# JuliaSmoothOptimizers/Krylov.jl

Measured on AMD Instinct MI355X. Metric: cg_iters_per_sec_poisson3d_csr_512cubed, higher is better.
Workload: dtype f64

## Files before the change

krylov.jl_amd/csrc/api.cpp:

```cpp
#include <cmath>
#include <cstdlib>

#include "khip_internal.hpp"

using namespace khip;

extern "C" int khip_comm_destroy_internal(khip_ctx *ctx);

namespace khip {
enum MapOpHost { H_COPY = 0, H_FILL, H_SCAL, H_SCALCOPY, H_DIVCOPY, H_AXPY, H_AXPBY, H_REF, H_WAXPY, H_VMUL, H_VDIV };
constexpr int kPadHost = 8;
}

namespace khip {
static int g_optional_build_failures = 0;
void optional_build(int rc) {
  if (rc == KHIP_OK) return;
  const hipError_t e = (hipError_t)take_hip_error();
  (void)hipGetLastError();
  if (e == hipErrorOutOfMemory || e == hipErrorMemoryAllocation) return;
  ++g_optional_build_failures;
  fprintf(stderr, "libkrylov_hip: an optional accelerator build failed (%d: %s; HIP: %s) -- falling back to the plain kernels\n", rc,
          khip_last_error(), hipGetErrorString(e));
}
// ... 100 lines not shown
  KHIP_CHECK_HIP(hipGetDeviceProperties(&prop, device));
  ctx->num_cu = prop.multiProcessorCount > 0 ? prop.multiProcessorCount : 256;
  KHIP_TRY(ensure_reduction_scratch(ctx, 1 << 18, 1));
  KHIP_CHECK_HIP(hipMalloc(&ctx->results, sizeof(double) * kResultSlots));
  KHIP_CHECK_HIP(hipMalloc(&ctx->results_dd, sizeof(dd) * kResultSlots));
  KHIP_CHECK_HIP(hipMemset(ctx->results, 0, sizeof(double) * kResultSlots));
  KHIP_CHECK_HIP(hipMemset(ctx->results_dd, 0, sizeof(dd) * kResultSlots));
  KHIP_CHECK_HIP(hipHostMalloc(reinterpret_cast<void **>(&ctx->results_pinned), sizeof(double) * kResultSlots * 2,
                               hipHostMallocDefault));
  *out = ctx;
  return KHIP_OK;
}

int khip_ctx_destroy(khip_ctx *ctx) {
  if (!ctx) return KHIP_OK;
  (void)hipSetDevice(ctx->device);
  (void)hipStreamSynchronize(ctx->stream);
  khip_comm_destroy_internal(ctx);
  panel_scratch_destroy(ctx);
  for (hipEvent_t e : ctx->prof_events) (void)hipEventDestroy(e);
  (void)hipFree(ctx->partials);
  (void)hipFree(ctx->partials2);
  (void)hipFree(ctx->tickets);
  (void)hipFree(ctx->results);
  (void)hipFree(ctx->results_dd);
  (void)hipHostFree(ctx->results_pinned);
  if (ctx->ev_fetch) (void)hipEventDestroy(ctx->ev_fetch);
  if (ctx->ev_red) (void)hipEventDestroy(ctx->ev_red);
  for (int i = 0; i < khip_ctx::kEvRing; ++i) {
    if (ctx->ev_a[i]) (void)hipEventDestroy(ctx->ev_a[i]);
    if (ctx->ev_b[i]) (void)hipEventDestroy(ctx->ev_b[i]);
  }
  if (ctx->comm_stream_hi && ctx->comm_stream_hi != ctx->comm_stream_lo) (void)hipStreamDestroy(ctx->comm_stream_hi);
  if (ctx->comm_stream_lo) (void)hipStreamDestroy(ctx->comm_stream_lo);
  if (ctx->own_stream) (void)hipStreamDestroy(ctx->stream);
  delete ctx;
  return KHIP_OK;
}

int khip_ctx_sync(khip_ctx *ctx) {
  KHIP_REQUIRE(ctx, "ctx_sync: null context");
  KHIP_CHECK_HIP(hipStreamSynchronize(ctx->stream));
  return KHIP_OK;
}

void *khip_ctx_stream(khip_ctx *ctx) { return ctx ? ctx->stream : nullptr; }

static int *tuning_field(khip_ctx *ctx, const char *key) {
  Tuning &t = ctx->tune;
  struct { const char *k; int *p; } tab[] = {
      {"spmv_kernel", &t.spmv_kernel}, {"spmv_rows", &t.spmv_rows}, {"spmv_vec", &t.spmv_vec},
      {"spmv_nt", &t.spmv_nt},         {"spmv_xcd", &t.spmv_xcd},   {"spmv_lanes", &t.spmv_lanes},
      {"compensated", &t.compensated}, {"nt_min_elems", &t.nt_min_elems}, {"overlap_halo", &t.overlap_halo},
      {"profile_spmv", &t.profile_spmv}, {"comm_priority", &t.comm_priority}, {"spmv_persist", &t.spmv_persist}, {"spmv_nty", &t.spmv_nty}, {"spmv_dot_early", &t.spmv_dot_early}, {"spmv_codes", &t.spmv_codes}, {"spmv_delta", &t.spmv_delta}, {"spmv_blk_pub", &t.spmv_blk_pub}, {"spmv_sell", &t.spmv_sell}, {"spmv_sell_narrow", &t.spmv_sell_narrow}, {"spmv_sell_entries", &t.spmv_sell_entries}, {"spmv_sell_pair", &t.spmv_sell_pair}, {"cg_setup_fused", &t.cg_setup_fused}, {"cg_defer_x", &t.cg_defer_x}, {"spmv_wide", &t.spmv_wide}, {"spmv_tiles", &t.spmv_tiles}, {"spmv_cap", &t.spmv_cap}, {"spmv_template", &t.spmv_template}, {"spmv_tmpl_rows", &t.spmv_tmpl_rows}, {"mgs_keep", &t.mgs_keep}, {"spmm_sweep", &t.spmm_sweep}, {"spmm_win_sweep", &t.spmm_win_sweep}, {"spmm_wide", &t.spmm_wide}, {"panel_fuse", &t.panel_fuse}, {"panel_signs", &t.panel_signs}, {"panel_qr_tsqr", &t.panel_qr_tsqr}, {"panel_a_lds", &t.panel_a_lds}, {"panel_nt", &t.panel_nt}, {"gmres_sstep", &t.gmres_sstep}, {"panel_multi_tiles", &t.panel_multi_tiles}, {"ilu_blocks", &t.ilu_blocks}, {"ilu_grid", &t.ilu_grid}, {"halo_mode", &t.halo_mode}, {"halo_gather_pct", &t.halo_gather_pct}, {"spmm_window", &t.spmm_window}, {"spmm_tile", &t.spmm_tile}, {"spmm_tile_exp", &t.spmm_tile_exp}, {"spmm_tile_nt", &t.spmm_tile_nt}, {"spmm_tile_slices", &t.spmm_tile_slices}, {"spmm_tile_pencil", &t.spmm_tile_pencil}, {"spmm_tile_slide", &t.spmm_tile_slide}, {"spmm_tile_ahead", &t.spmm_tile_ahead}, {"spmm_tile_xcd", &t.spmm_tile_xcd}, {"spmm_tile_dbuf", &t.spmm_tile_dbuf}, {"spmm_tile_pair", &t.spmm_tile_pair}, {"spmm_tile_waves", &t.spmm_tile_waves}, {"spmm_tile_grid", &t.spmm_tile_grid}, {"spmm_tile_shape", &t.spmm_tile_shape}, {"spmm_window_grid", &t.spmm_window_grid}, {"spmm_sweep_s", &t.spmm_sweep_s}, {"spmm_sweep_w", &t.spmm_sweep_w}, {"red_u", &t.red_u}, {"hist_window", &t.hist_window}};
  for (auto &e : tab)
    if (strcmp(e.k, key) == 0) return e.p;
  return nullptr;
}

int khip_ctx_set_option(khip_ctx *ctx, const char *key, int value) {
  KHIP_REQUIRE(ctx && key, "set_option: null argument");
  int *p = tuning_field(ctx, key);
  KHIP_REQUIRE(p, "set_option: unknown key '%s'", key);
  *p = value;
  if (p == &ctx->tune.comm_priority) {
    KHIP_CHECK_HIP(hipStreamSynchronize(ctx->stream));
    KHIP_CHECK_HIP(hipStreamSynchronize(ctx->comm_stream_hi));
    KHIP_CHECK_HIP(hipStreamSynchronize(ctx->comm_stream_lo));
    ctx->comm_stream = value ? ctx->comm_stream_hi : ctx->comm_stream_lo;
  }
  return KHIP_OK;
}

int khip_ctx_get_option(khip_ctx *ctx, const char *key, int *value) {
  KHIP_REQUIRE(ctx && key && value, "get_option: null argument");
  int *p = tuning_field(ctx, key);
  KHIP_REQUIRE(p, "get_option: unknown key '%s'", key);
  *value = *p;
  return KHIP_OK;
}

int khip_malloc(khip_ctx *ctx, size_t bytes, void **dptr) {
  KHIP_REQUIRE(ctx && dptr, "malloc: null argument");
  KHIP_CHECK_HIP(hipSetDevice(ctx->device));
  *dptr = nullptr;
  if (bytes == 0) return KHIP_OK;
  KHIP_CHECK_HIP(hipMalloc(dptr, bytes));
  return KHIP_OK;
}

int khip_free(khip_ctx *ctx, void *dptr) {
  KHIP_REQUIRE(ctx, "free: null context");
  if (!dptr) return KHIP_OK;
  KHIP_CHECK_HIP(hipStreamSynchronize(ctx->stream));
  KHIP_CHECK_HIP(hipFree(dptr));
  return KHIP_OK;
}

int khip_memcpy_h2d(khip_ctx *ctx, void *dst, const void *src_host, size_t bytes) {
  KHIP_REQUIRE(ctx && (bytes == 0 || (dst && src_host)), "memcpy_h2d: null argument");
  if (!bytes) return KHIP_OK;
  KHIP_CHECK_HIP(hipMemcpyAsync(dst, src_host, bytes, hipMemcpyHostToDevice, ctx->stream));
  KHIP_CHECK_HIP(hipStreamSynchronize(ctx->stream));
  return KHIP_OK;
}

int khip_memcpy_d2h(khip_ctx *ctx, void *dst_host, const void *src, size_t bytes) {
// ... 563 lines not shown
```

krylov.jl_amd/csrc/device_reduce.hpp:

```cpp
#pragma once

#include <hip/hip_runtime.h>

#include "khip_internal.hpp"
#include "solver_device.hpp"

namespace khip {

typedef double dbl2 __attribute__((ext_vector_type(2)));
template <int VEC> struct VecT;
template <> struct VecT<1> { using type = double; };
template <> struct VecT<2> { using type = dbl2; };

__device__ __forceinline__ double vget(const double &v, int) { return v; }
__device__ __forceinline__ double vget(const dbl2 &v, int i) { return i == 0 ? v.x : v.y; }
__device__ __forceinline__ void vset(double &v, int, double s) { v = s; }
__device__ __forceinline__ void vset(dbl2 &v, int i, double s) { if (i == 0) v.x = s; else v.y = s; }

template <bool NT, typename T> __device__ __forceinline__ T ldg(const T *p) {
  if (NT) return __builtin_nontemporal_load(p);
  return *p;
}
template <bool NT, typename T> __device__ __forceinline__ void stg(T v, T *p) {
  if (NT) __builtin_nontemporal_store(v, p);
// ... 40 lines not shown
__device__ __forceinline__ double dpp_f64(double v) {
  int lo = __double2loint(v), hi = __double2hiint(v);
  lo = __builtin_amdgcn_update_dpp(0, lo, CTRL, ROW_MASK, 0xf, false);
  hi = __builtin_amdgcn_update_dpp(0, hi, CTRL, ROW_MASK, 0xf, false);
  return __hiloint2double(hi, lo);
}
template <int CTRL, int ROW_MASK>
__device__ __forceinline__ dd dpp_step(dd v) {
  dd o;
  o.hi = dpp_f64<CTRL, ROW_MASK>(v.hi);
  o.lo = dpp_f64<CTRL, ROW_MASK>(v.lo);
  return dd_merge(v, o);
}

constexpr int kResultLane = 63;

__device__ __forceinline__ dd wave_reduce(dd v) {
#ifdef KHIP_REDUCE_SHFL
#pragma unroll
  for (int off = 1; off < 64; off <<= 1) {
    dd o;
    o.hi = __shfl_up(v.hi, off, 64);
    o.lo = __shfl_up(v.lo, off, 64);
    if ((int)(threadIdx.x & 63) < off) o = dd{0.0, 0.0};
    v = dd_merge(v, o);
  }
  return v;
#endif
  v = dpp_step<0x111, 0xf>(v);
  v = dpp_step<0x112, 0xf>(v);
  v = dpp_step<0x114, 0xf>(v);
  v = dpp_step<0x118, 0xf>(v);
  v = dpp_step<0x142, 0xa>(v);
  v = dpp_step<0x143, 0xc>(v);
  return v;
}

struct RedArgs {
  dd *wave_partials;
  dd *blk_partials;
  unsigned *ticket;
  double *results;
  dd *results_dd;
  int64_t cap;
  int64_t wave_offset;
  int slot;
  const long long *stop_seq;
  long long seq;
  int epi;
  void *epi_state;
};

template <int NOUT>
__device__ __forceinline__ void wave_publish(dd (&acc)[NOUT], const RedArgs &ra) {
  const int64_t wid = ra.wave_offset + (int64_t)blockIdx.x * (blockDim.x >> 6) + (threadIdx.x >> 6);
#pragma unroll
  for (int o = 0; o < NOUT; ++o) {
    dd r = wave_reduce(acc[o]);
    if ((threadIdx.x & 63) == kResultLane) ra.wave_partials[(size_t)o * ra.cap + wid] = r;
  }
}

template <int NOUT>
__device__ __forceinline__ void block_publish(dd (&acc)[NOUT], const RedArgs &ra, dd *s_red) {
  const int tid = threadIdx.x, lane = tid & 63, wave = tid >> 6;
  const int64_t wid = ra.wave_offset + (int64_t)blockIdx.x * (blockDim.x >> 6) + wave;
#pragma unroll
  for (int o = 0; o < NOUT; ++o) s_red[o * kBlock + tid] = acc[o];
  __syncthreads();
  if (wave == 0) {
#pragma unroll
    for (int o = 0; o < NOUT; ++o) {
      dd v = s_red[o * kBlock + lane];
      v = dd_merge(v, s_red[o * kBlock + 64 + lane]);
      v = dd_merge(v, s_red[o * kBlock + 128 + lane]);
      v = dd_merge(v, s_red[o * kBlock + 192 + lane]);
      v = wave_reduce(v);
      if (lane == kResultLane) ra.wave_partials[(size_t)o * ra.cap + wid] = v;
    }
  } else if (lane == kResultLane) {
#pragma unroll
    for (int o = 0; o < NOUT; ++o) ra.wave_partials[(size_t)o * ra.cap + wid] = dd{0.0, 0.0};
  }
}

template <int NOUT>
__device__ __forceinline__ void block_reduce(dd (&acc)[NOUT], dd (*s_w)[kWavesPerBlock]) {
  const int lane = threadIdx.x & 63, wave = threadIdx.x >> 6;
#pragma unroll
  for (int o = 0; o < NOUT; ++o) {
    dd r = wave_reduce(acc[o]);
    if (lane == kResultLane) s_w[o][wave] = r;
  }
  __syncthreads();
  if (threadIdx.x == 0) {
#pragma unroll
    for (int o = 0; o < NOUT; ++o) {
      dd t = s_w[o][0];
#pragma unroll
      for (int w = 1; w < kWavesPerBlock; ++w) t = dd_merge(t, s_w[o][w]);
      acc[o] = t;
    }
  }
}

template <int NOUT>
__global__ __launch_bounds__(kBlock) void reduce_finish_kernel(RedArgs ra, int64_t P) {
  __shared__ dd s_w[NOUT][kWavesPerBlock];
  __shared__ int s_last;
  if (seq_skip(ra.stop_seq, ra.seq)) return;
  const int G = gridDim.x;
  const int64_t chunk = (P + G - 1) / G;
  const int64_t lo = chunk * blockIdx.x;
  const int64_t hi = (lo + chunk < P) ? lo + chunk : P;
  dd acc[NOUT];
#pragma unroll
  for (int o = 0; o < NOUT; ++o) {
    dd a = {0.0, 0.0};
    const dd *src = ra.wave_partials + (size_t)o * ra.cap;
    for (int64_t base = lo + threadIdx.x; base < hi; base += (int64_t)kBlock * 8) {
      dd v[8];
#pragma unroll
      for (int j = 0; j < 8; ++j) {
        const int64_t i = base + (int64_t)j * kBlock;
        v[j] = src[i < hi ? i : base];
      }
#pragma unroll
      for (int j = 0; j < 8; ++j)
        if (base + (int64_t)j * kBlock < hi) a = dd_merge(a, v[j]);
    }
    acc[o] = a;
  }
  block_reduce<NOUT>(acc, s_w);
  if (G == 1) {
    if (threadIdx.x == 0) {
#pragma unroll
      for (int o = 0; o < NOUT; ++o) {
// ... 65 lines not shown
```

krylov.jl_amd/csrc/khip_internal.hpp:

```cpp
#pragma once

#include <hip/hip_runtime.h>

#include <unistd.h>

#include <chrono>
#include <cstdarg>
#include <cstdint>
#include <cstdio>
#include <cstring>
#include <string>
#include <vector>

#include "../../include/krylov_hip.h"

namespace khip {

void set_error(const char *fmt, ...);
void note_hip_error(int e);
int take_hip_error();

inline void klogf(int fd, const char *fmt, ...) {
  va_list ap;
  va_start(ap, fmt);
// ... 8 lines not shown
    hipError_t e__ = (expr);                                                              \
    if (e__ != hipSuccess) {                                                              \
      ::khip::note_hip_error((int)e__);                                                   \
      ::khip::set_error("%s failed: %s (%s:%d)", #expr, hipGetErrorString(e__), __FILE__, \
                        __LINE__);                                                        \
      return KHIP_ERR_HIP;                                                                \
    }                                                                                     \
  } while (0)

#define KHIP_REQUIRE(cond, ...)          \
  do {                                   \
    if (!(cond)) {                       \
      ::khip::set_error(__VA_ARGS__);    \
      return KHIP_ERR_INVALID;           \
    }                                    \
  } while (0)

#define KHIP_TRY(expr)                 \
  do {                                 \
    int rc__ = (expr);                 \
    if (rc__ != KHIP_OK) return rc__;  \
  } while (0)

struct dd {
  double hi, lo;
};

__host__ __device__ inline double dd_value(double hi, double lo) { return __builtin_isfinite(hi) ? hi + lo : hi; }

constexpr int kMaxNout = 4;
constexpr int kMaxRedOut = 64;
constexpr int kResultSlots = 256;

struct Comm;

struct Tuning {
  int spmv_kernel = 0;
  int spmv_rows = 256;
  int spmv_vec = 1;
  int spmv_nt = 0;
  int spmv_xcd = 0;
  int spmv_nty = -1;
  int spmv_dot_early = 0;
  int spmv_tiles = 1;
  int spmv_template = 1;
  int spmv_tmpl_rows = 8;
  int spmv_cap = 0;
  int cg_defer_x = 1;
  int cg_setup_fused = 1;
  int spmv_sell = 2;
  int spmv_sell_pair = 1;
  int spmv_sell_entries = 1;
  int spmv_sell_narrow = 0;
  int spmv_blk_pub = 0;
  int spmv_delta = 0;
  int spmv_wide = 0;
  int spmv_codes = 1;
  int spmv_lanes = 0;
  int spmv_persist = 0;
  int compensated = 1;
  int nt_min_elems = 1 << 22;
  int mgs_keep = -1;
  int hist_window = 1 << 14;
  int red_u = 0;
  int ilu_blocks = 1;
  int ilu_grid = 0;
  int panel_multi_tiles = 2;
  int gmres_sstep = 4;
  int panel_nt = 0;
  int panel_a_lds = 1;
  int panel_qr_tsqr = 0;
  int panel_signs = 1;
  int panel_fuse = 1;
  int spmm_wide = 1;
  int spmm_window_grid = 0;
  int spmm_tile = 1;
  int spmm_tile_exp = 0;
  int spmm_tile_waves = 0;
  int spmm_tile_grid = 0;
  int spmm_tile_pair = 1;
  int spmm_tile_dbuf = -1;
  int spmm_tile_xcd = -1;
  int spmm_tile_ahead = 0;
  int spmm_tile_slide = -1;
  int spmm_tile_pencil = 0;
  int spmm_tile_slices = 0;
  int spmm_tile_nt = 0;
  int spmm_tile_shape = 0;
  int spmm_window = 1;
  int spmm_sweep = 0;
  int spmm_win_sweep = 0;
  int spmm_sweep_s = 0;
  int spmm_sweep_w = 64;
  int overlap_halo = 1;
  int halo_mode = 0;
  int halo_gather_pct = 50;
  int halo_self = 0;
  int comm_priority = 1;
  int profile_spmv = 0;
};

struct SeqCtl {
  const long long *stop_seq = nullptr;
  long long seq = 0;
  int epi = 0;
  void *epi_state = nullptr;
};

struct LanczosEpi {
  const double *coef = nullptr;
  const double *r1 = nullptr;
  int sub_r1 = 0;
};

}

namespace khip {
enum SpmmLast {
  kSlFamily = 0,
  kSlL, kSlNL, kSlDbuf, kSlAhead, kSlRunLen, kSlGrid, kSlXcd, kSlLaunches, kSlDirect,
  kSlSweepS, kSlSweepW, kSlSweepK, kSlSweepCols, kSlNt, kSlDist, kSlP, kSlPow2, kSlBlock, kSlLds, kSlNumCu,
  kSpmmLastWords = 24
};
}

struct khip_ctx {
  int device = 0;
  hipStream_t stream = nullptr;
  bool own_stream = false;
  hipStream_t comm_stream = nullptr;
  hipStream_t comm_stream_hi = nullptr, comm_stream_lo = nullptr;
  static constexpr int kEvRing = 16;
  hipEvent_t ev_a[kEvRing] = {}, ev_b[kEvRing] = {};
  unsigned ev_cur = 0;
  hipEvent_t ev_fetch = nullptr;
  hipEvent_t ev_red = nullptr;
  bool allreduce_pending = false;
  int num_cu = 256;
  int64_t spmm_last[khip::kSpmmLastWords] = {};
  khip::dd *partials = nullptr;
  khip::dd *partials2 = nullptr;
  unsigned *tickets = nullptr;
  int64_t red_cap1 = 0;
  int *scratch_word = nullptr;
  double *results = nullptr;
  khip::dd *results_dd = nullptr;
  double *results_pinned = nullptr;
  int next_slot = 0;
  khip::Tuning tune;
  khip::SeqCtl ctl;
  khip::LanczosEpi lz;
  khip::Comm *comm = nullptr;
  void *panel_scratch = nullptr;
  std::vector<hipEvent_t> prof_events;
  std::vector<int> prof_tags;
  int prof_spmv_tag = 0;
  size_t prof_used = 0;
};

struct khip_csr {
  khip_ctx *ctx = nullptr;
  int64_t m = 0, n = 0, nnz = 0;
  int32_t *rowptr = nullptr;
  int32_t *blockptr = nullptr;
  int32_t *col = nullptr;
  double *val = nullptr;
  int64_t max_row_nnz = 0;
  int64_t band = 0;
  int64_t plane_rows = 0;
  int64_t line_rows = 0;
  double mean_row_nnz = 0;
  bool dist = false;
  int64_t n_global = 0, row0 = 0;
  int64_t n_ghost = 0;
  double *ghost = nullptr;
  double *sendbuf = nullptr;
  int32_t *send_idx = nullptr;
  double *ghost_w = nullptr, *sendbuf_w = nullptr;
  int halo_w_cap = 0;
  int64_t n_send = 0;
  std::vector<int64_t> send_off, recv_off;
  std::vector<int64_t> part_starts;
  std::vector<int32_t> ghost_gid;
  bool self_halo = false;
  bool gather = false;
  int64_t gather_maxm = 0;
  std::vector<int64_t> gather_rows;
  int64_t interior_lo = 0, interior_hi = 0;
  uint16_t *tmpl_id = nullptr;
  int32_t *tmpl_off = nullptr;
  double *tmpl_val = nullptr;
// ... 222 lines not shown
```

krylov.jl_amd/csrc/spmv.hip:

```cpp
#include "spmv_common.hpp"

#ifndef KHIP_STAGE_AUX
#define KHIP_STAGE_AUX 2
#endif

namespace khip {

__device__ __forceinline__ void store_y(const SpmvArgs &a, int64_t row, double v) {
  if (a.nt_y == 2) {
    const double *p = a.y + row;
    asm volatile("global_store_dwordx2 %0, %1, off sc1\n\ts_nop 1" :: "v"(p), "v"(v) : "memory");
  } else if (a.nt_y) __builtin_nontemporal_store(v, a.y + row);
  else a.y[row] = v;
}

__device__ __forceinline__ int chunk_id(int b, int G, int xcd_run) {
  if (xcd_run > 0) {
    const int win = 8 * xcd_run;
    const int full = (G / win) * win;
    if (b < full) return (b / win) * win + (b & 7) * xcd_run + ((b % win) >> 3);
    return b;
  }
  if (xcd_run < 0 && (G & 7) == 0) return (b & 7) * (G >> 3) + (b >> 3);
  return b;
// ... 290 lines not shown
#pragma unroll
          for (int u = 0; u < UK; ++u) {
            xx[u] = 0.0;
            if (k0 + u < hi) xx[u] = gather_x<DIST>(a, cc[u]);
          }
#pragma unroll
          for (int u = 0; u < UK; ++u) {
            if (k0 + u < hi) {
              const double prod = vv[u] * xx[u];
              acc = acc + prod;
            }
          }
        }
      }
      __syncthreads();
    }
    if (tid < nr) {
      store_y(a, r0 + tid, acc);
      if (DOT) {
        if (!a.dot_early) wv = a.dotw[r0 + tid];
        acc_prod<COMP>(dacc[0], wv, acc);
        if (a.dot_sq == 1) acc_prod<COMP>(dacc[1], acc, acc);
        else if (a.dot_sq == 2) acc_prod<COMP>(dacc[1], wv, wv);
      }
    }
  }
  if (DOT) {
    if (a.blk_pub) {
      dd *s_red = reinterpret_cast<dd *>(s_stage);
      if (a.dot_sq) block_publish<2>(dacc, ra, s_red);
      else block_publish<1>(reinterpret_cast<dd (&)[1]>(dacc), ra, s_red);
    } else if (a.dot_sq) wave_publish<2>(dacc, ra);
    else wave_publish<1>(reinterpret_cast<dd (&)[1]>(dacc), ra);
  }
}


template <bool DIST>
__device__ __forceinline__ double ent_step(const SpmvArgs &a, int32_t row, unsigned long long cw, const int32_t *s_off, const double *s_val, double acc) {
  double vv[8], xx[8];
  int32_t cc[8];
  bool on[8];
#pragma unroll
  for (int u = 0; u < 8; ++u) { const int c = (int)((cw >> (8 * u)) & 0xFFull); on[u] = c != 0xFF; cc[u] = row + s_off[c]; vv[u] = s_val[c]; }
#pragma unroll
  for (int u = 0; u < 8; ++u) {
    xx[u] = 0.0;
    if (on[u]) xx[u] = gather_x<DIST>(a, cc[u]);
  }
#pragma unroll
  for (int u = 0; u < 8; ++u) {
    if (on[u]) {
      const double prod = vv[u] * xx[u];
      acc = acc + prod;
    }
  }
  return acc;
}

template <bool NTM>
__device__ __forceinline__ dbl2 ent_first(const SpmvArgs &a, int64_t rowl, int64_t o0, int T) {
  dbl2 ce = dbl2{0.0, 0.0};
  if (T == 1) ce.x = __longlong_as_double((long long)ld<NTM>(a.sell + (size_t)o0 * 64 + (rowl & 63)));
  else if (T > 1) ce = ld<NTM>(reinterpret_cast<const dbl2 *>(a.sell + (size_t)o0 * 64) + (rowl & 63));
  return ce;
}

template <bool DOT, bool COMP, bool DIST, bool NTM, bool COLS32, bool C4, bool PAIR, bool PAIRG, bool ENT = false>
__global__ __launch_bounds__(kBlock) void spmv_sell_kernel(SpmvArgs a, RedArgs ra) {
  if (seq_skip(a.stop_seq, a.seq)) return;
  const int ROWS = a.stage_rows;
  extern __shared__ __attribute__((aligned(16))) unsigned char s_stage[];
  const size_t pub = (DOT && a.blk_pub) ? sizeof(dd) * (size_t)kBlock * (a.dot_sq ? 2u : 1u) : 0u;
  int32_t *s_tab = reinterpret_cast<int32_t *>(s_stage + pub);
  double *s_val = reinterpret_cast<double *>(s_stage + pub + 256 * sizeof(int32_t));
  const int tid = threadIdx.x;
  const int64_t nrows = a.row_hi - a.row_lo - a.hole_len;
  const int64_t nrb = (nrows + ROWS - 1) / ROWS;
  const int tpb = a.tiles_per_block > 0 ? a.tiles_per_block : 1;
  const int cid = chunk_id(blockIdx.x, gridDim.x, a.xcd_remap);
  const int64_t rb_begin = (int64_t)cid * tpb;
  const int64_t rb_end = (rb_begin + tpb < nrb) ? rb_begin + tpb : nrb;
  dd dacc[2];
  dacc[0] = dd{0.0, 0.0};
  dacc[1] = dd{0.0, 0.0};
  dbl2 ent_next = dbl2{0.0, 0.0};
  auto ent_prefetch = [&](int64_t rb) {
    if (rb >= rb_end || tid >= ROWS) return;
    int64_t rn = a.row_lo + rb * ROWS;
    if (rn >= a.hole_lo) rn += a.hole_len;
    rn += tid;
    if (rn >= a.row_hi) return;
    const int64_t sn = rn >> 6;
    int64_t on;
    int Tn;
    if (a.sell_units) { on = sn * a.sell_units; Tn = a.sell_units; }
    else { const uint32_t b0 = a.sell_off[sn], b1 = a.sell_off[sn + 1]; on = (int64_t)b0; Tn = (int)(b1 - b0); }
    ent_next = ent_first<NTM>(a, rn, on, Tn);
  };
  if (ENT) {
    const int32_t *eo = static_cast<const int32_t *>(a.sell_ent);
    const double *ev = reinterpret_cast<const double *>(eo + 256);
    ent_prefetch(rb_begin);
    for (int i = tid; i < 256; i += kBlock) { s_tab[i] = eo[i]; s_val[i] = ev[i]; }
    __syncthreads();
  } else if (!COLS32) {
// ... 101 lines not shown
        bool on[8];
        if (COLS32) {
#pragma unroll
          for (int j = 0; j < 4; ++j) {
            const unsigned long long cw = (2 * j < left) ? ld<NTM>(base + (size_t)(k0 / 2 + j) * 64) : ~0ull;
            cc[2 * j] = (int32_t)(uint32_t)(cw & 0xFFFFFFFFull);
            cc[2 * j + 1] = (int32_t)(uint32_t)(cw >> 32);
          }
#pragma unroll
          for (int u = 0; u < 8; ++u) on[u] = cc[u] != -1;
        } else if (C4) {
          const uint32_t cw = ld<NTM>(a.sell_c4 + rowl);
#pragma unroll
          for (int u = 0; u < 8; ++u) { const int c = (int)((cw >> (4 * u)) & 0xFu); on[u] = c != 0xF; cc[u] = row + s_tab[c]; }
        } else {
          const unsigned long long cw = ld<NTM>(base + (size_t)(k0 / 8) * 64);
#pragma unroll
          for (int u = 0; u < 8; ++u) { const int c = (int)((cw >> (8 * u)) & 0xFFull); on[u] = c != 0xFF; cc[u] = row + s_tab[c]; }
        }
#pragma unroll
        for (int u = 0; u < 8; ++u) vv[u] = (u < left) ? __longlong_as_double((long long)ld<NTM>(vb + (size_t)u * 64)) : 0.0;
#pragma unroll
        for (int u = 0; u < 8; ++u) {
          xx[u] = 0.0;
          if (on[u]) xx[u] = gather_x<DIST>(a, cc[u]);
        }
#pragma unroll
        for (int u = 0; u < 8; ++u) {
          if (on[u]) {
            const double prod = vv[u] * xx[u];
            acc = acc + prod;
          }
        }
      }
      if (DOT && a.lz) acc = lanczos_row(a, rowl, acc, wv);
      store_y(a, rowl, acc);
      if (DOT) {
        acc_prod<COMP>(dacc[0], wv, acc);
        if (a.dot_sq == 1) acc_prod<COMP>(dacc[1], acc, acc);
        else if (a.dot_sq == 2) acc_prod<COMP>(dacc[1], wv, wv);
      }
    }
  }
  if (DOT) {
    if (a.blk_pub) {
      dd *s_red = reinterpret_cast<dd *>(s_stage);
      if (a.dot_sq) block_publish<2>(dacc, ra, s_red);
      else block_publish<1>(reinterpret_cast<dd (&)[1]>(dacc), ra, s_red);
    } else if (a.dot_sq) wave_publish<2>(dacc, ra);
    else wave_publish<1>(reinterpret_cast<dd (&)[1]>(dacc), ra);
  }
}

template <> struct code_load<int32_t> {
  typedef u32x4 vec;
  template <int AUX = 0>
  static __device__ __forceinline__ vec ld(__amdgpu_buffer_rsrc_t r, int byte_off) {
    return __builtin_amdgcn_raw_buffer_load_b128(r, byte_off, 0, AUX);
  }
};

template <typename CODE, bool DOT, bool COMP, bool DIST>
__global__ __launch_bounds__(kBlock) void spmv_delta_kernel(SpmvArgs a, RedArgs ra) {
  if (seq_skip(a.stop_seq, a.seq)) return;
  typedef typename code_load<CODE>::vec cvec;
  constexpr bool PLAIN = sizeof(CODE) == 4;
  constexpr unsigned ESC = PLAIN ? 0xffffffffu : ((1u << (8 * (sizeof(CODE) & 3))) - 1u);
  constexpr int CAP = 2048;
  __shared__ __attribute__((aligned(16))) double s_prod[CAP + 8];
  const int ROWS = a.stage_rows;
  const int tid = threadIdx.x;
  const CODE *code = reinterpret_cast<const CODE *>(PLAIN ? (const void *)a.col : a.dcode);
  const int64_t nrows = a.row_hi - a.row_lo;
  const int64_t nrb = (nrows + ROWS - 1) / ROWS;
  const int G = gridDim.x;
  const int cid = chunk_id(blockIdx.x, G, a.xcd_remap);
  const int64_t rb_begin = nrb * cid / G;
  const int64_t rb_end = nrb * (cid + 1) / G;
  dd dacc[2];
  dacc[0] = dd{0.0, 0.0};
  dacc[1] = dd{0.0, 0.0};

  for (int64_t rb = rb_begin; rb < rb_end; ++rb) {
    const int64_t r0 = a.row_lo + rb * ROWS;
    const int nr = (int)((a.row_hi - r0) < ROWS ? (a.row_hi - r0) : ROWS);
    const int64_t s = a.rowptr[r0], e = a.rowptr[r0 + nr];
    const int my_a = (tid < nr) ? a.rowptr[r0 + tid] : 0;
    const int my_b = (tid < nr) ? a.rowptr[r0 + tid + 1] : 0;
    int32_t base = 0, E0 = 0, E1 = 0;
    if (!PLAIN) {
      const int64_t bi = r0 / ROWS;
      base = a.dbase[bi];
      E0 = a.desc_ptr[bi];
      E1 = a.desc_ptr[bi + 1];
    }
    double acc = 0.0, wv = 0.0;
    if (DOT && a.dot_early && tid < nr) wv = a.dotw[r0 + tid];
    for (int64_t c0 = s & ~(int64_t)3; c0 < e; c0 += CAP) {
      const int lim = (int)((e - c0) < (int64_t)CAP ? (e - c0) : (int64_t)CAP);
      const int lim4 = (lim + 3) & ~3;
      const int first = (int)(s - c0) > 0 ? (int)(s - c0) : 0;
      const __amdgpu_buffer_rsrc_t rv =
          __builtin_amdgcn_make_buffer_rsrc(const_cast<double *>(a.val + c0), 0, lim4 * 8, kBufRsrcWord3);
      const __amdgpu_buffer_rsrc_t rc =
          __builtin_amdgcn_make_buffer_rsrc(const_cast<CODE *>(code + c0), 0, lim4 * (int)sizeof(CODE), kBufRsrcWord3);
      u32x4 v[4];
// ... 351 lines not shown
      if (dist) LAUNCH(false, false, true); else LAUNCH(false, false, false);            \
    }                                                                                    \
  } while (0)

template <int ROWS, int VEC, bool NT>
static void launch_stream_cfg(khip_ctx *ctx, const SpmvArgs &a, const RedArgs &ra, unsigned grid, bool dot, bool comp,
                              bool dist) {
#define KHIP_L(DOT, COMP, DIST) \
  hipLaunchKernelGGL((spmv_stream_kernel<ROWS, VEC, NT, DOT, COMP, DIST>), dim3(grid), dim3(kBlock), 0, ctx->stream, a, ra)
  KHIP_DISPATCH_DCD(KHIP_L);
#undef KHIP_L
}

template <int ROWS, bool NT>
static void launch_stage_cfg(khip_ctx *ctx, const SpmvArgs &a, const RedArgs &ra, unsigned grid, bool dot, bool comp,
                             bool dist) {
  size_t lds = 12u * (size_t)a.stage_cap;
  const size_t pub = dot && a.blk_pub ? sizeof(dd) * (size_t)kBlock * (a.dot_sq ? 2u : 1u) : 0u;
  if (lds < pub) lds = pub;
#define KHIP_L(DOT, COMP, DIST) \
  hipLaunchKernelGGL((spmv_stage_kernel<ROWS, NT, DOT, COMP, DIST>), dim3(grid), dim3(kBlock), lds, ctx->stream, a, ra)
  KHIP_DISPATCH_DCD(KHIP_L);
#undef KHIP_L
}

template <typename CODE>
static void launch_code_cfg(khip_ctx *ctx, const SpmvArgs &a, const RedArgs &ra, unsigned grid, bool dot, bool comp,
                            bool dist) {
  size_t lds = (8u + sizeof(CODE)) * (size_t)a.stage_cap + 4u * (size_t)a.code_T;
  const size_t pub = dot && a.blk_pub ? sizeof(dd) * (size_t)kBlock * (a.dot_sq ? 2u : 1u) : 0u;
  if (lds < pub) lds = pub;
#define KHIP_L(DOT, COMP, DIST) \
  hipLaunchKernelGGL((spmv_code_kernel<CODE, DOT, COMP, DIST>), dim3(grid), dim3(kBlock), lds, ctx->stream, a, ra)
  KHIP_DISPATCH_DCD(KHIP_L);
#undef KHIP_L
}

static void launch_sell_cfg(khip_ctx *ctx, const SpmvArgs &a, const RedArgs &ra, unsigned grid, bool dot, bool comp, bool dist) {
  const size_t pub = dot && a.blk_pub ? sizeof(dd) * (size_t)kBlock * (a.dot_sq ? 2u : 1u) : 0u;
  const size_t lds = pub + 4u * 256u + (a.sell_ent ? 8u * 256u : 0u);
#define KHIP_SELL(DOT, COMP, DIST, NTM, COLS32, C4) \
  do { if (a.sell_ent) hipLaunchKernelGGL((spmv_sell_kernel<DOT, COMP, DIST, NTM, false, false, false, false, true>), dim3(grid), dim3(kBlock), lds, ctx->stream, a, ra); \
       else if (a.sell_pair == 1) hipLaunchKernelGGL((spmv_sell_kernel<DOT, COMP, DIST, NTM, false, false, true, false>), dim3(grid), dim3(kBlock), lds, ctx->stream, a, ra); \
       else if (a.sell_pair == 2) hipLaunchKernelGGL((spmv_sell_kernel<DOT, COMP, DIST, NTM, COLS32, false, false, true>), dim3(grid), dim3(kBlock), lds, ctx->stream, a, ra); \
       else hipLaunchKernelGGL((spmv_sell_kernel<DOT, COMP, DIST, NTM, COLS32, C4, false, false>), dim3(grid), dim3(kBlock), lds, ctx->stream, a, ra); } while (0)
#define KHIP_L(DOT, COMP, DIST) \
  do { const bool ntm = ctx->tune.spmv_sell == 2; \
       if (a.sell_cols) { if (ntm) KHIP_SELL(DOT, COMP, DIST, true, true, false); else KHIP_SELL(DOT, COMP, DIST, false, true, false); } \
       else if (a.sell_c4) { if (ntm) KHIP_SELL(DOT, COMP, DIST, true, false, true); else KHIP_SELL(DOT, COMP, DIST, false, false, true); } \
       else { if (ntm) KHIP_SELL(DOT, COMP, DIST, true, false, false); else KHIP_SELL(DOT, COMP, DIST, false, false, false); } } while (0)
  KHIP_DISPATCH_DCD(KHIP_L);
#undef KHIP_L
#undef KHIP_SELL
}

template <typename CODE>
static void launch_delta_cfg(khip_ctx *ctx, const SpmvArgs &a, const RedArgs &ra, unsigned grid, bool dot, bool comp,
                             bool dist) {
#define KHIP_L(DOT, COMP, DIST) \
  hipLaunchKernelGGL((spmv_delta_kernel<CODE, DOT, COMP, DIST>), dim3(grid), dim3(kBlock), 0, ctx->stream, a, ra)
  KHIP_DISPATCH_DCD(KHIP_L);
#undef KHIP_L
}

static void launch_wave_cfg(khip_ctx *ctx, const SpmvArgs &a, const RedArgs &ra, unsigned grid, bool dot, bool comp, bool dist) {
  const size_t lds = 12u * (size_t)a.stage_cap;
#define KHIP_L(DOT, COMP, DIST) \
  hipLaunchKernelGGL((spmv_wave_kernel<DOT, COMP, DIST>), dim3(grid), dim3(64), lds, ctx->stream, a, ra)
  KHIP_DISPATCH_DCD(KHIP_L);
#undef KHIP_L
}

template <int L, int RPG, bool NT>
static void launch_ordered_cfg(khip_ctx *ctx, const SpmvArgs &a, const RedArgs &ra, unsigned grid, bool dot, bool comp,
                               bool dist) {
#define KHIP_L(DOT, COMP, DIST) \
  hipLaunchKernelGGL((spmv_ordered_kernel<L, RPG, NT, DOT, COMP, DIST>), dim3(grid), dim3(kBlock), 0, ctx->stream, a, ra)
  KHIP_DISPATCH_DCD(KHIP_L);
#undef KHIP_L
}

template <int LPR>
static void launch_vector_cfg(khip_ctx *ctx, const SpmvArgs &a, const RedArgs &ra, unsigned grid, bool dot, bool comp,
                              bool dist) {
#define KHIP_L(DOT, COMP, DIST) \
  hipLaunchKernelGGL((spmv_vector_kernel<LPR, DOT, COMP, DIST>), dim3(grid), dim3(kBlock), 0, ctx->stream, a, ra)
  KHIP_DISPATCH_DCD(KHIP_L);
#undef KHIP_L
}

static void launch_template_cfg(khip_ctx *ctx, const SpmvArgs &a, const RedArgs &ra, unsigned grid, bool dot, bool comp,
                                bool dist) {
  const size_t lds = (size_t)a.tmpl_T * a.tmpl_K * 12 + (size_t)a.tmpl_T * 4;
#define KHIP_L(DOT, COMP, DIST) \
  hipLaunchKernelGGL((spmv_template_kernel<DOT, COMP, DIST>), dim3(grid), dim3(kBlock), lds, ctx->stream, a, ra)
  KHIP_DISPATCH_DCD(KHIP_L);
#undef KHIP_L
}

static inline unsigned pick_grid(khip_ctx *ctx, int64_t tiles, bool persist) {
  if (tiles < 1) tiles = 1;
  if (persist) {
    int64_t cap = (int64_t)ctx->num_cu * 8;
    int64_t g = tiles < cap ? tiles : cap;
    if (g >= 8) g &= ~(int64_t)7;
    return (unsigned)g;
// ... 158 lines not shown
    if (dot) KHIP_TRY(ensure_reduction_scratch(ctx, *wave_cursor + (int64_t)grid * kWavesPerBlock, nout));
    ra = make_red_args(ctx, dot ? dot_slot : 0); ra.wave_offset = *wave_cursor;
    launch_template_cfg(ctx, a, ra, grid, dot, comp, dist);
  } else if (form == SpmvForm::Stream) {
    const int rows = plan.rows;
    const bool delta = plan.delta && row_lo % A->delta_rows == 0;
    if (delta || plan.wide) {
      a.stage_rows = delta ? A->delta_rows : rows;
      if (delta) { a.dcode = A->dcode; a.dbase = A->dbase; a.desc_ptr = A->desc_ptr; a.desc_pos = A->desc_pos; a.desc_col = A->desc_col; }
      grid = pick_grid(ctx, (nrows + a.stage_rows - 1) / a.stage_rows, false);
      if (dot) KHIP_TRY(ensure_reduction_scratch(ctx, *wave_cursor + (int64_t)grid * kWavesPerBlock, nout));
      ra = make_red_args(ctx, dot ? dot_slot : 0); ra.wave_offset = *wave_cursor;
      if (!delta) launch_delta_cfg<int32_t>(ctx, a, ra, grid, dot, comp, dist);
      else if (A->delta_bits == 8) launch_delta_cfg<uint8_t>(ctx, a, ra, grid, dot, comp, dist);
      else launch_delta_cfg<uint16_t>(ctx, a, ra, grid, dot, comp, dist);
    } else {
      grid = pick_grid(ctx, (nrows + rows - 1) / rows, persist);
      if (dot) KHIP_TRY(ensure_reduction_scratch(ctx, *wave_cursor + (int64_t)grid * kWavesPerBlock, nout));
      ra = make_red_args(ctx, dot ? dot_slot : 0); ra.wave_offset = *wave_cursor;
      const int vec = ctx->tune.spmv_vec == 2 ? 2 : 1;
#define KHIP_ROWS(R)                                                                              \
  do {                                                                                            \
    if (vec == 2) { if (nt) launch_stream_cfg<R, 2, true>(ctx, a, ra, grid, dot, comp, dist);     \
                    else    launch_stream_cfg<R, 2, false>(ctx, a, ra, grid, dot, comp, dist); }  \
    else          { if (nt) launch_stream_cfg<R, 1, true>(ctx, a, ra, grid, dot, comp, dist);     \
                    else    launch_stream_cfg<R, 1, false>(ctx, a, ra, grid, dot, comp, dist); }  \
  } while (0)
      switch (rows) {
        case 256: KHIP_ROWS(256); break;
        case 128: KHIP_ROWS(128); break;
        case 64: KHIP_ROWS(64); break;
        default: KHIP_ROWS(32); break;
      }
#undef KHIP_ROWS
    }
  } else if (plan.staged_family()) {
    const int rows = plan.rows;
    const int64_t nrb = (nrows + rows - 1) / rows;
    a.tiles_per_block = ctx->tune.spmv_tiles > 0 ? ctx->tune.spmv_tiles : ((dot && nrb >= 8192) ? 2 : 1);
    {
      int64_t cap = ctx->tune.spmv_cap > 0 ? ctx->tune.spmv_cap : (int64_t)rows * A->max_row_nnz + 3;
      cap = (cap + 3) & ~(int64_t)3;
      a.stage_cap = (int)(cap < 64 ? 64 : (cap > 2048 ? 2048 : cap));
    }
    grid = pick_grid(ctx, (nrb + a.tiles_per_block - 1) / a.tiles_per_block, false);
    if ((int64_t)grid * a.tiles_per_block < nrb) a.tiles_per_block = (int)((nrb + grid - 1) / grid);
    if (dot) KHIP_TRY(ensure_reduction_scratch(ctx, *wave_cursor + (int64_t)grid * kWavesPerBlock, nout));
    ra = make_red_args(ctx, dot ? dot_slot : 0); ra.wave_offset = *wave_cursor;
    a.stage_rows = rows;
    if (form == SpmvForm::Sliced || form == SpmvForm::Coded) { a.code = A->code; a.code_tab = A->code_tab; a.code_T = A->code_T; }
    if (form == SpmvForm::Sliced) {
      a.sell = A->sell; a.sell_off = A->sell_off; a.sell_units = A->sell_units; a.sell_cols = 0; a.sell_c4 = A->sell_c4; a.sell_pair = A->sell_pair;
      a.sell_ent = A->sell_ent_state == 1 ? A->sell_ent_tab : nullptr;
      launch_sell_cfg(ctx, a, ra, grid, dot, comp, dist);
    } else if (form == SpmvForm::Sliced32) {
      a.sell = A->sell32; a.sell_off = A->sell32_off; a.sell_units = A->sell32_units; a.sell_cols = 1; a.sell_pair = A->sell32_pair; a.sell_c4 = nullptr;
      launch_sell_cfg(ctx, a, ra, grid, dot, comp, dist);
    } else if (form == SpmvForm::Coded) {
      if (A->code_bits == 8) launch_code_cfg<uint8_t>(ctx, a, ra, grid, dot, comp, dist);
      else launch_code_cfg<uint16_t>(ctx, a, ra, grid, dot, comp, dist);
    } else {
#define KHIP_STG(R) do { if (nt) launch_stage_cfg<R, true>(ctx, a, ra, grid, dot, comp, dist); \
                         else launch_stage_cfg<R, false>(ctx, a, ra, grid, dot, comp, dist); } while (0)
      switch (rows) {
        case 256: KHIP_STG(256); break;
        case 128: KHIP_STG(128); break;
        case 64: KHIP_STG(64); break;
        default: KHIP_STG(32); break;
      }
#undef KHIP_STG
    }
  } else if (form == SpmvForm::Ordered) {
    int L = ctx->tune.spmv_lanes;
    if (L == 0) {
      L = 4;
      const double target = A->max_row_nnz <= 64 ? (double)A->max_row_nnz : A->mean_row_nnz;
      while (L < 64 && L < target) L <<= 1;
    }
#define KHIP_ORD(LL, RPG)                                                                     \
  do {                                                                                        \
    constexpr int rpb = (64 / LL) * RPG * kWavesPerBlock;                                     \
    grid = pick_grid(ctx, (nrows + rpb - 1) / rpb, persist);                                  \
    if (dot) KHIP_TRY(ensure_reduction_scratch(ctx, *wave_cursor + (int64_t)grid * kWavesPerBlock, nout));                                \
    ra = make_red_args(ctx, dot ? dot_slot : 0); ra.wave_offset = *wave_cursor;                                              \
    if (nt) launch_ordered_cfg<LL, RPG, true>(ctx, a, ra, grid, dot, comp, dist);             \
    else launch_ordered_cfg<LL, RPG, false>(ctx, a, ra, grid, dot, comp, dist);               \
  } while (0)
    switch (L) {
      case 4: KHIP_ORD(4, 4); break;
      case 8: KHIP_ORD(8, 4); break;
      case 16: KHIP_ORD(16, 4); break;
      case 32: KHIP_ORD(32, 2); break;
      default: KHIP_ORD(64, 1); break;
    }
#undef KHIP_ORD
  } else {
    int lpr = ctx->tune.spmv_lanes;
    if (lpr == 0) {
      lpr = 4;
      while (lpr < 64 && lpr * 2 <= A->mean_row_nnz) lpr <<= 1;
    }
    const int rpb = kBlock / lpr;
    grid = pick_grid(ctx, (nrows + rpb - 1) / rpb, persist);
    if (dot) KHIP_TRY(ensure_reduction_scratch(ctx, *wave_cursor + (int64_t)grid * kWavesPerBlock, nout));
    ra = make_red_args(ctx, dot ? dot_slot : 0); ra.wave_offset = *wave_cursor;
    switch (lpr) {
      case 4: launch_vector_cfg<4>(ctx, a, ra, grid, dot, comp, dist); break;
// ... 17 lines not shown
```

Baseline: 383.2.

## Add persistent SELL SpMV kernel with prefetched entry codes across row blocks

New measurement: 414.7 (median of 6 runs). 8.2% higher.

```diff
diff --git a/krylov.jl_amd/csrc/api.cpp b/krylov.jl_amd/csrc/api.cpp
--- a/krylov.jl_amd/csrc/api.cpp
+++ b/krylov.jl_amd/csrc/api.cpp
@@ -176,7 +176,7 @@
       {"spmv_kernel", &t.spmv_kernel}, {"spmv_rows", &t.spmv_rows}, {"spmv_vec", &t.spmv_vec},
       {"spmv_nt", &t.spmv_nt},         {"spmv_xcd", &t.spmv_xcd},   {"spmv_lanes", &t.spmv_lanes},
       {"compensated", &t.compensated}, {"nt_min_elems", &t.nt_min_elems}, {"overlap_halo", &t.overlap_halo},
-      {"profile_spmv", &t.profile_spmv}, {"comm_priority", &t.comm_priority}, {"spmv_persist", &t.spmv_persist}, {"spmv_nty", &t.spmv_nty}, {"spmv_dot_early", &t.spmv_dot_early}, {"spmv_codes", &t.spmv_codes}, {"spmv_delta", &t.spmv_delta}, {"spmv_blk_pub", &t.spmv_blk_pub}, {"spmv_sell", &t.spmv_sell}, {"spmv_sell_narrow", &t.spmv_sell_narrow}, {"spmv_sell_entries", &t.spmv_sell_entries}, {"spmv_sell_pair", &t.spmv_sell_pair}, {"cg_setup_fused", &t.cg_setup_fused}, {"cg_defer_x", &t.cg_defer_x}, {"spmv_wide", &t.spmv_wide}, {"spmv_tiles", &t.spmv_tiles}, {"spmv_cap", &t.spmv_cap}, {"spmv_template", &t.spmv_template}, {"spmv_tmpl_rows", &t.spmv_tmpl_rows}, {"mgs_keep", &t.mgs_keep}, {"spmm_sweep", &t.spmm_sweep}, {"spmm_win_sweep", &t.spmm_win_sweep}, {"spmm_wide", &t.spmm_wide}, {"panel_fuse", &t.panel_fuse}, {"panel_signs", &t.panel_signs}, {"panel_qr_tsqr", &t.panel_qr_tsqr}, {"panel_a_lds", &t.panel_a_lds}, {"panel_nt", &t.panel_nt}, {"gmres_sstep", &t.gmres_sstep}, {"panel_multi_tiles", &t.panel_multi_tiles}, {"ilu_blocks", &t.ilu_blocks}, {"ilu_grid", &t.ilu_grid}, {"halo_mode", &t.halo_mode}, {"halo_gather_pct", &t.halo_gather_pct}, {"spmm_window", &t.spmm_window}, {"spmm_tile", &t.spmm_tile}, {"spmm_tile_exp", &t.spmm_tile_exp}, {"spmm_tile_nt", &t.spmm_tile_nt}, {"spmm_tile_slices", &t.spmm_tile_slices}, {"spmm_tile_pencil", &t.spmm_tile_pencil}, {"spmm_tile_slide", &t.spmm_tile_slide}, {"spmm_tile_ahead", &t.spmm_tile_ahead}, {"spmm_tile_xcd", &t.spmm_tile_xcd}, {"spmm_tile_dbuf", &t.spmm_tile_dbuf}, {"spmm_tile_pair", &t.spmm_tile_pair}, {"spmm_tile_waves", &t.spmm_tile_waves}, {"spmm_tile_grid", &t.spmm_tile_grid}, {"spmm_tile_shape", &t.spmm_tile_shape}, {"spmm_window_grid", &t.spmm_window_grid}, {"spmm_sweep_s", &t.spmm_sweep_s}, {"spmm_sweep_w", &t.spmm_sweep_w}, {"red_u", &t.red_u}, {"hist_window", &t.hist_window}};
+      {"profile_spmv", &t.profile_spmv}, {"comm_priority", &t.comm_priority}, {"spmv_persist", &t.spmv_persist}, {"spmv_nty", &t.spmv_nty}, {"spmv_dot_early", &t.spmv_dot_early}, {"spmv_codes", &t.spmv_codes}, {"spmv_delta", &t.spmv_delta}, {"spmv_blk_pub", &t.spmv_blk_pub}, {"spmv_sell", &t.spmv_sell}, {"spmv_sell_narrow", &t.spmv_sell_narrow}, {"spmv_sell_entries", &t.spmv_sell_entries}, {"spmv_sell_persist", &t.spmv_sell_persist}, {"spmv_sell_pair", &t.spmv_sell_pair}, {"cg_setup_fused", &t.cg_setup_fused}, {"cg_defer_x", &t.cg_defer_x}, {"spmv_wide", &t.spmv_wide}, {"spmv_tiles", &t.spmv_tiles}, {"spmv_cap", &t.spmv_cap}, {"spmv_template", &t.spmv_template}, {"spmv_tmpl_rows", &t.spmv_tmpl_rows}, {"mgs_keep", &t.mgs_keep}, {"spmm_sweep", &t.spmm_sweep}, {"spmm_win_sweep", &t.spmm_win_sweep}, {"spmm_wide", &t.spmm_wide}, {"panel_fuse", &t.panel_fuse}, {"panel_signs", &t.panel_signs}, {"panel_qr_tsqr", &t.panel_qr_tsqr}, {"panel_a_lds", &t.panel_a_lds}, {"panel_nt", &t.panel_nt}, {"gmres_sstep", &t.gmres_sstep}, {"panel_multi_tiles", &t.panel_multi_tiles}, {"ilu_blocks", &t.ilu_blocks}, {"ilu_grid", &t.ilu_grid}, {"halo_mode", &t.halo_mode}, {"halo_gather_pct", &t.halo_gather_pct}, {"spmm_window", &t.spmm_window}, {"spmm_tile", &t.spmm_tile}, {"spmm_tile_exp", &t.spmm_tile_exp}, {"spmm_tile_nt", &t.spmm_tile_nt}, {"spmm_tile_slices", &t.spmm_tile_slices}, {"spmm_tile_pencil", &t.spmm_tile_pencil}, {"spmm_tile_slide", &t.spmm_tile_slide}, {"spmm_tile_ahead", &t.spmm_tile_ahead}, {"spmm_tile_xcd", &t.spmm_tile_xcd}, {"spmm_tile_dbuf", &t.spmm_tile_dbuf}, {"spmm_tile_pair", &t.spmm_tile_pair}, {"spmm_tile_waves", &t.spmm_tile_waves}, {"spmm_tile_grid", &t.spmm_tile_grid}, {"spmm_tile_shape", &t.spmm_tile_shape}, {"spmm_window_grid", &t.spmm_window_grid}, {"spmm_sweep_s", &t.spmm_sweep_s}, {"spmm_sweep_w", &t.spmm_sweep_w}, {"red_u", &t.red_u}, {"hist_window", &t.hist_window}};
   for (auto &e : tab)
     if (strcmp(e.k, key) == 0) return e.p;
   return nullptr;
diff --git a/krylov.jl_amd/csrc/device_reduce.hpp b/krylov.jl_amd/csrc/device_reduce.hpp
--- a/krylov.jl_amd/csrc/device_reduce.hpp
+++ b/krylov.jl_amd/csrc/device_reduce.hpp
@@ -116,19 +116,21 @@
 };
 
 template <int NOUT>
-__device__ __forceinline__ void wave_publish(dd (&acc)[NOUT], const RedArgs &ra) {
-  const int64_t wid = ra.wave_offset + (int64_t)blockIdx.x * (blockDim.x >> 6) + (threadIdx.x >> 6);
+__device__ __forceinline__ void wave_publish_at(dd (&acc)[NOUT], const RedArgs &ra, int64_t blk) {
+  const int64_t wid = ra.wave_offset + blk * (blockDim.x >> 6) + (threadIdx.x >> 6);
 #pragma unroll
   for (int o = 0; o < NOUT; ++o) {
     dd r = wave_reduce(acc[o]);
     if ((threadIdx.x & 63) == kResultLane) ra.wave_partials[(size_t)o * ra.cap + wid] = r;
   }
 }
-
-template <int NOUT>
-__device__ __forceinline__ void block_publish(dd (&acc)[NOUT], const RedArgs &ra, dd *s_red) {
+template <int NOUT>
+__device__ __forceinline__ void wave_publish(dd (&acc)[NOUT], const RedArgs &ra) { wave_publish_at<NOUT>(acc, ra, (int64_t)blockIdx.x); }
+
+template <int NOUT>
+__device__ __forceinline__ void block_publish_at(dd (&acc)[NOUT], const RedArgs &ra, dd *s_red, int64_t blk) {
   const int tid = threadIdx.x, lane = tid & 63, wave = tid >> 6;
-  const int64_t wid = ra.wave_offset + (int64_t)blockIdx.x * (blockDim.x >> 6) + wave;
+  const int64_t wid = ra.wave_offset + blk * (blockDim.x >> 6) + wave;
 #pragma unroll
   for (int o = 0; o < NOUT; ++o) s_red[o * kBlock + tid] = acc[o];
   __syncthreads();
@@ -147,6 +149,9 @@
     for (int o = 0; o < NOUT; ++o) ra.wave_partials[(size_t)o * ra.cap + wid] = dd{0.0, 0.0};
   }
 }
+
+template <int NOUT>
+__device__ __forceinline__ void block_publish(dd (&acc)[NOUT], const RedArgs &ra, dd *s_red) { block_publish_at<NOUT>(acc, ra, s_red, (int64_t)blockIdx.x); }
 
 template <int NOUT>
 __device__ __forceinline__ void block_reduce(dd (&acc)[NOUT], dd (*s_w)[kWavesPerBlock]) {
diff --git a/krylov.jl_amd/csrc/khip_internal.hpp b/krylov.jl_amd/csrc/khip_internal.hpp
--- a/krylov.jl_amd/csrc/khip_internal.hpp
+++ b/krylov.jl_amd/csrc/khip_internal.hpp
@@ -84,6 +84,7 @@
   int spmv_sell_pair = 1;
   int spmv_sell_entries = 1;
   int spmv_sell_narrow = 0;
+  int spmv_sell_persist = 1;
   int spmv_blk_pub = 0;
   int spmv_delta = 0;
   int spmv_wide = 0;
@@ -169,6 +170,7 @@
   hipEvent_t ev_red = nullptr;
   bool allreduce_pending = false;
   int num_cu = 256;
+  int sell_persist_occ[32][3] = {};
   int64_t spmm_last[khip::kSpmmLastWords] = {};
   khip::dd *partials = nullptr;
   khip::dd *partials2 = nullptr;
diff --git a/krylov.jl_amd/csrc/spmv.hip b/krylov.jl_amd/csrc/spmv.hip
--- a/krylov.jl_amd/csrc/spmv.hip
+++ b/krylov.jl_amd/csrc/spmv.hip
@@ -366,6 +366,28 @@
   for (int u = 0; u < 8; ++u) {
     if (on[u]) {
       const double prod = vv[u] * xx[u];
+      acc = acc + prod;
+    }
+  }
+  return acc;
+}
+
+template <bool DIST>
+__device__ __forceinline__ double ent_step_late(const SpmvArgs &a, int32_t row, unsigned long long cw, const int32_t *s_off, const double *s_val, double acc) {
+  double xx[8];
+  int32_t cc[8];
+#pragma unroll
+  for (int u = 0; u < 8; ++u) cc[u] = row + s_off[(int)((cw >> (8 * u)) & 0xFFull)];
+#pragma unroll
+  for (int u = 0; u < 8; ++u) {
+    xx[u] = 0.0;
+    if (((cw >> (8 * u)) & 0xFFull) != 0xFFull) xx[u] = gather_x<DIST>(a, cc[u]);
+  }
+#pragma unroll
+  for (int u = 0; u < 8; ++u) {
+    const int c = (int)((cw >> (8 * u)) & 0xFFull);
+    if (c != 0xFF) {
+      const double prod = s_val[c] * xx[u];
       acc = acc + prod;
     }
   }
@@ -573,6 +595,112 @@
   }
 }
 
+struct SellPos { int v, rb, rb_end; };
+
+template <bool DOT, bool COMP, bool DIST, bool NTM, bool ONE>
+__global__ __launch_bounds__(kBlock) void spmv_sell_persist_kernel(SpmvArgs a, RedArgs ra, int nvirt) {
+  if (seq_skip(a.stop_seq, a.seq)) return;
+  const int ROWS = a.stage_rows;
+  extern __shared__ __attribute__((aligned(16))) unsigned char s_stage[];
+  const size_t pub = (DOT && a.blk_pub) ? sizeof(dd) * (size_t)kBlock * (a.dot_sq ? 2u : 1u) : 0u;
+  int32_t *s_off = reinterpret_cast<int32_t *>(s_stage + 2 * pub);
+  double *s_val = reinterpret_cast<double *>(s_stage + 2 * pub + 256 * sizeof(int32_t));
+  const int tid = threadIdx.x;
+  const int G = gridDim.x;
+  const int64_t nrows = a.row_hi - a.row_lo - a.hole_len;
+  const int nrb = (int)((nrows + ROWS - 1) / ROWS);
+  const int tpb = a.tiles_per_block > 0 ? a.tiles_per_block : 1;
+  auto first_of = [&](int v) -> SellPos {
+    if (v >= nvirt) return SellPos{v, nrb, nrb};
+    const int64_t b = (int64_t)chunk_id(v, nvirt, a.xcd_remap) * tpb;
+    return SellPos{v, (int)(b < nrb ? b : nrb), (int)((b + tpb < nrb) ? b + tpb : nrb)};
+  };
+  auto next_of = [&](const SellPos &p) -> SellPos {
+    if (p.rb + 1 < p.rb_end) return SellPos{p.v, p.rb + 1, p.rb_end};
+    return first_of(p.v + G);
+  };
+  auto lane_row = [&](const SellPos &p) -> int64_t {
+    if (p.rb >= p.rb_end || tid >= ROWS) return -1;
+    int64_t r = a.row_lo + (int64_t)p.rb * ROWS;
+    if (r >= a.hole_lo) r += a.hole_len;
+    r += tid;
+    return r < a.row_hi ? r : -1;
+  };
+  auto slice_of = [&](int64_t rowl, int64_t &o0, int &T) {
+    const int64_t sl = rowl >> 6;
+    if (ONE) { o0 = sl; T = 1; }
+    else if (a.sell_units) { o0 = sl * a.sell_units; T = a.sell_units; }
+    else { const uint32_t b0 = a.sell_off[sl], b1 = a.sell_off[sl + 1]; o0 = (int64_t)b0; T = (int)(b1 - b0); }
+  };
+  auto load_codes = [&](const SellPos &p, dbl2 &ce) {
+    const int64_t rowl = lane_row(p);
+    if (rowl < 0) return;
+    int64_t o0;
+    int T;
+    slice_of(rowl, o0, T);
+    ce = ent_first<NTM>(a, rowl, o0, T);
+  };
+  auto walk_row = [&](int64_t rowl, dbl2 ce) -> double {
+    int64_t o0;
+    int T;
+    slice_of(rowl, o0, T);
+    const dbl2 *pb = reinterpret_cast<const dbl2 *>(a.sell + (size_t)o0 * 64) + (rowl & 63);
+    double acc = 0.0;
+    for (int w = 0; w < T; ++w) {
+      if (w >= 2 && (w & 1) == 0) ce = ld<NTM>(pb + (size_t)(w >> 1) * 64);
+      acc = ent_step_late<DIST>(a, (int32_t)rowl, (unsigned long long)__double_as_longlong((w & 1) ? ce.y : ce.x), s_off, s_val, acc);
+    }
+    return acc;
+  };
+  dd dacc[2];
+  dacc[0] = dd{0.0, 0.0};
+  dacc[1] = dd{0.0, 0.0};
+  auto finish_row = [&](int64_t rowl, double acc, double wv) {
+    if (DOT && a.lz) acc = lanczos_row(a, rowl, acc, wv);
+    store_y(a, rowl, acc);
+    if (DOT) {
+      acc_prod<COMP>(dacc[0], wv, acc);
+      if (a.dot_sq == 1) acc_prod<COMP>(dacc[1], acc, acc);
+      else if (a.dot_sq == 2) acc_prod<COMP>(dacc[1], wv, wv);
+    }
+  };
+  int npub = 0;
+  auto publish = [&](int v) {
+    if (DOT) {
+      if (a.blk_pub) {
+        dd *s_red = reinterpret_cast<dd *>(s_stage + (size_t)(npub & 1) * pub);
+        if (a.dot_sq) block_publish_at<2>(dacc, ra, s_red, v);
+        else block_publish_at<1>(reinterpret_cast<dd (&)[1]>(dacc), ra, s_red, v);
+      } else if (a.dot_sq) wave_publish_at<2>(dacc, ra, v);
+      else wave_publish_at<1>(reinterpret_cast<dd (&)[1]>(dacc), ra, v);
+      ++npub;
+      dacc[0] = dd{0.0, 0.0};
+      dacc[1] = dd{0.0, 0.0};
+    }
+  };
+
+  SellPos cur = first_of(blockIdx.x);
+  dbl2 ent_next = dbl2{0.0, 0.0};
+  load_codes(cur, ent_next);
+  {
+    const int32_t *eo = static_cast<const int32_t *>(a.sell_ent);
+    const double *ev = reinterpret_cast<const double *>(eo + 256);
+    for (int i = tid; i < 256; i += kBlock) { s_off[i] = eo[i]; s_val[i] = ev[i]; }
+    __syncthreads();
+  }
+  while (cur.v < nvirt) {
+    const SellPos nxt = next_of(cur);
+    const int64_t rowl = lane_row(cur);
+    double wv = 0.0;
+    if (DOT && rowl >= 0) wv = a.dotw[rowl];
+    const dbl2 ce = ent_next;
+    load_codes(nxt, ent_next);
+    if (rowl >= 0) finish_row(rowl, walk_row(rowl, ce), wv);
+    if (nxt.v != cur.v) publish(cur.v);
+    cur = nxt;
+  }
+}
+
 template <> struct code_load<int32_t> {
   typedef u32x4 vec;
   template <int AUX = 0>
@@ -1030,6 +1158,35 @@
   KHIP_DISPATCH_DCD(KHIP_L);
 #undef KHIP_L
 #undef KHIP_SELL
+}
+
+constexpr int kSellPersistRounds = 8;
+static bool launch_sell_persist_cfg(khip_ctx *ctx, const SpmvArgs &a, const RedArgs &ra, unsigned nvirt, int want, bool dot, bool comp, bool dist) {
+  const size_t pub = dot && a.blk_pub ? sizeof(dd) * (size_t)kBlock * (a.dot_sq ? 2u : 1u) : 0u;
+  const size_t lds = 2u * pub + 4u * 256u + 8u * 256u;
+  const bool ntm = ctx->tune.spmv_sell == 2;
+  unsigned grid = 0;
+  bool ok = true;
+#define KHIP_L(DOT, COMP, DIST) \
+  do { auto go = [&](auto kern, int key) { \
+         if (want > 1) grid = (unsigned)want < nvirt ? (unsigned)want : nvirt; \
+         else if (a.sell_units != 1) { ok = false; return; } \
+         else { \
+           int &nb = ctx->sell_persist_occ[key][pub ? (a.dot_sq ? 2 : 1) : 0]; \
+           if (nb == 0 && (hipOccupancyMaxActiveBlocksPerMultiprocessor(&nb, kern, kBlock, lds) != hipSuccess || nb <= 0)) { (void)hipGetLastError(); nb = -1; } \
+           const int64_t g = nb > 0 ? ((int64_t)nb * ctx->num_cu * kSellPersistRounds) & ~(int64_t)7 : 0; \
+           if (g < 8 || (int64_t)nvirt <= g) { ok = false; return; } \
+           grid = (unsigned)g; \
+         } \
+         hipLaunchKernelGGL(kern, dim3(grid), dim3(kBlock), lds, ctx->stream, a, ra, (int)nvirt); }; \
+       const int key = (DOT ? 1 : 0) | (COMP ? 2 : 0) | (DIST ? 4 : 0) | (ntm ? 8 : 0); \
+       if (a.sell_units == 1) { if (ntm) go(spmv_sell_persist_kernel<DOT, COMP, DIST, true, true>, key | 16); \
+                                else go(spmv_sell_persist_kernel<DOT, COMP, DIST, false, true>, key | 16); } \
+       else if (ntm) go(spmv_sell_persist_kernel<DOT, COMP, DIST, true, false>, key); \
+       else go(spmv_sell_persist_kernel<DOT, COMP, DIST, false, false>, key); } while (0)
+  KHIP_DISPATCH_DCD(KHIP_L);
+#undef KHIP_L
+  return ok;
 }
 
 template <typename CODE>
@@ -1294,7 +1451,9 @@
     if (form == SpmvForm::Sliced) {
       a.sell = A->sell; a.sell_off = A->sell_off; a.sell_units = A->sell_units; a.sell_cols = 0; a.sell_c4 = A->sell_c4; a.sell_pair = A->sell_pair;
       a.sell_ent = A->sell_ent_state == 1 ? A->sell_ent_tab : nullptr;
-      launch_sell_cfg(ctx, a, ra, grid, dot, comp, dist);
+      const int want = ctx->tune.spmv_sell_persist;
+      if (!(a.sell_ent && want > 0 && launch_sell_persist_cfg(ctx, a, ra, grid, want, dot, comp, dist)))
+        launch_sell_cfg(ctx, a, ra, grid, dot, comp, dist);
     } else if (form == SpmvForm::Sliced32) {
       a.sell = A->sell32; a.sell_off = A->sell32_off; a.sell_units = A->sell32_units; a.sell_cols = 1; a.sell_pair = A->sell32_pair; a.sell_c4 = nullptr;
       launch_sell_cfg(ctx, a, ra, grid, dot, comp, dist);
```
